# ZechengLi19/CIM

Measured on AMD Instinct MI355X. Metric: images/sec training step (ResNet-50 VOC, ~1k proposals/img) at 1/2/4/8 GPU, higher is better.
Workload: dtype fp32

## Files before the change

### cim_amd/csrc/conv1x1.hip

```cpp
#include "common.h"
#include "../../include/cim_hip.h"

#ifndef CIM_BODY_PRIO_LEVEL
#define CIM_BODY_PRIO_LEVEL 3
#endif
#if CIM_BODY_PRIO_LEVEL > 0
#define CIM_BODY_PRIO() __builtin_amdgcn_s_setprio(CIM_BODY_PRIO_LEVEL)
#else
#define CIM_BODY_PRIO()
#endif
namespace {

#ifndef CIM_SMALL_BK
#define CIM_SMALL_BK 32
#endif
#ifndef CIM_SMALL_ABL
#define CIM_SMALL_ABL 0
#endif
constexpr int SBM = 64, SBN = 64, SBK = CIM_SMALL_BK;
constexpr int SLD = 68;
typedef float f32x16 __attribute__((ext_vector_type(16)));
typedef float f32x4u __attribute__((ext_vector_type(4), aligned(4)));
__device__ __forceinline__ float4 ld4(const float* p) {
    const f32x4u v = *reinterpret_cast<const f32x4u*>(p);
    return make_float4(v.x, v.y, v.z, v.w);
}

struct SmallArgs {
    const float* A; const float* B; float* C; float* Xraw;
    const float* gamma; const float* beta; const float* mean; const float* var; const float* res;
    float eps;
    int M, N, K, lda, ldb, ldc;
    int a_mcontig, b_kcontig, relu, bn;
    int splits; float* ws;
    const float* colbias;
    const float* mask; const float* mgamma; const float* mvar; float meps;
    const float* mxr; const float* mmean; float* mpart; int mparts;
    int res_w, res_ws, res_hw;
};
struct InputBn { const float* y; const float* gamma; const float* var; float eps;
                 const float* xr; const float* mean; float* part; };

typedef unsigned int u32x4 __attribute__((ext_vector_type(4)));
typedef __amdgpu_buffer_rsrc_t rsrc_t;
__device__ __forceinline__ rsrc_t make_rsrc(const float* p, long long floats) {
    return __builtin_amdgcn_make_buffer_rsrc(const_cast<float*>(p), 0, (int)(unsigned)(floats * 4), 0x00020000);
}
__device__ __forceinline__ float4 bld4(rsrc_t r, unsigned byte_off) {
    const u32x4 v = __builtin_amdgcn_raw_buffer_load_b128(r, byte_off, 0, 0);
    return make_float4(__uint_as_float(v.x), __uint_as_float(v.y), __uint_as_float(v.z), __uint_as_float(v.w));
}
__device__ __forceinline__ float bld1(rsrc_t r, unsigned byte_off) {
    return __uint_as_float(__builtin_amdgcn_raw_buffer_load_b32(r, byte_off, 0, 0));
}
constexpr unsigned OOB = 0x7fffffffu;
__host__ __device__ __forceinline__ long long tile_extent(bool RC, int rows, int K, int ld) {
    return RC ? (long long)(K - 1) * ld + rows : (long long)(rows - 1) * ld + K;
}
template <bool RC, int ROWS>
__device__ __forceinline__ unsigned tile_off(int ld, int r0, int k0, int p) {
    int r, k;
    if (RC) { k = k0 + p / (ROWS / 4); r = r0 + (p % (ROWS / 4)) * 4; return ((unsigned)k * ld + r) * 4u; }
    r = r0 + p % ROWS; k = k0 + (p / ROWS) * 4;
    return ((unsigned)r * ld + k) * 4u;
}
template <bool RC, int ROWS>
__device__ __forceinline__ float4 tile_ktail(float4 v, int K, int k0, int p) {
    if (!RC) {
        const int left = K - (k0 + (p / ROWS) * 4);
        v.x = left > 0 ? v.x : 0.0f; v.y = left > 1 ? v.y : 0.0f; v.z = left > 2 ? v.z : 0.0f; v.w = left > 3 ? v.w : 0.0f;
    }
    return v;
}

template <bool RC, int ROWS>
__device__ __forceinline__ void tile_store(float* __restrict__ S, float4 v, int p) {
    if (RC) {
        const int k = p / (ROWS / 4), r = (p % (ROWS / 4)) * 4;
        *reinterpret_cast<float4*>(S + k * SLD + r) = v;
    } else {
        const int r = p % ROWS, k = (p / ROWS) * 4;
        S[(k + 0) * SLD + r] = v.x;
        S[(k + 1) * SLD + r] = v.y;
        S[(k + 2) * SLD + r] = v.z;
        S[(k + 3) * SLD + r] = v.w;
    }
}

__device__ __forceinline__ float small_value(const SmallArgs& g, int row, int col, float v, float& s1, float& s2) {
    const size_t o = (size_t)row * g.ldc + col;
    float y = v;
    if (g.bn) {
        const float a = g.gamma[row] * rsqrtf(g.var[row] + g.eps);
        y = fmaf(v, a, g.beta[row] - g.mean[row] * a);
    }
    if (g.res) {
        if (g.res_w == 0) y += g.res[o];
        else {
            const int py = col / g.res_w, px = col - py * g.res_w;
            if (!((py | px) & 1)) y += g.res[(size_t)row * g.res_hw + (py >> 1) * g.res_ws + (px >> 1)];
        }
    }
    if (g.colbias) y += g.colbias[col];
    if (g.relu) y = fmaxf(y, 0.0f);
    if (g.mask) {
        const bool on = g.mask[o] > 0.0f;
        if (g.mpart && on) { s1 += y; s2 = fmaf(y, g.mxr[o] - g.mmean[row], s2); }
        y = on ? y * (g.mgamma[row] * rsqrtf(g.mvar[row] + g.meps)) : 0.0f;
// ... 59 lines not shown
#pragma unroll
            for (int r = 0; r < 16; ++r) {
                const int row = row0 + 8 * (r >> 2) + 4 * (lane >> 5) + (r & 3);
                if (row < g.M) small_finish(g, row, col, acc[r]);
            }
        }
        return;
    }
#pragma unroll
    for (int r = 0; r < 16; ++r) {
        const int row = row0 + 8 * (r >> 2) + 4 * (lane >> 5) + (r & 3);
        float s1 = 0.0f, s2 = 0.0f;
        if (cm.in(nc) && row < g.M) small_finish(g, row, col, acc[r], s1, s2);
        small_put_part(g, row, cm.group(col0), lane, s1, s2);
    }
}


template <bool AM, bool BKc, int WN>
__global__ __launch_bounds__(128 * WN) void gemm_small_kernel(const SmallArgs g) {
    CIM_BODY_PRIO();
    constexpr int NT = 128 * WN, BNT = 32 * WN;
    constexpr int PA = SBM * 8 / NT, PB = BNT * 8 / NT;
    __shared__ __attribute__((aligned(16))) float As[2][SBK * SLD];
    __shared__ __attribute__((aligned(16))) float Bs[2][SBK * SLD];
    const int tid = threadIdx.x, lane = tid & 63, wave = tid >> 6;
    const int wm = wave / WN, wn = wave % WN;
    const int tiles_n = (g.N + BNT - 1) / BNT;
    const int tile = blockIdx.x;
    const int m0 = (tile / tiles_n) * SBM, n0 = (tile % tiles_n) * BNT;
    const int split = blockIdx.y;
    const int kper = ((g.K + g.splits - 1) / g.splits + SBK - 1) / SBK * SBK;
    const int kbeg = split * kper, kend = min(g.K, kbeg + kper);
#if CIM_SMALL_ABL == 4
    if (g.M > 0) return;
#endif

    f32x16 acc;
#pragma unroll
    for (int i = 0; i < 16; ++i) acc[i] = 0.0f;

    const rsrc_t RA_ = make_rsrc(g.A, tile_extent(AM, g.M, g.K, g.lda)), RB_ = make_rsrc(g.B, tile_extent(!BKc, g.N, g.K, g.ldb));
    unsigned oa[PA], ob[PB];
#pragma unroll
    for (int i = 0; i < PA; ++i) oa[i] = tile_off<AM, SBM>(g.lda, m0, kbeg, tid + i * NT);
#pragma unroll
    for (int i = 0; i < PB; ++i) ob[i] = tile_off<!BKc, BNT>(g.ldb, n0, kbeg, tid + i * NT);
    const unsigned sa = (AM ? (unsigned)g.lda * SBK : (unsigned)SBK) * 4u, sb = (!BKc ? (unsigned)g.ldb * SBK : (unsigned)SBK) * 4u;
    float4 ra0[PA], rb0[PB], ra1[PA], rb1[PB];
#if CIM_SMALL_ABL == 3
#define SM_GLOAD(RA, RB, S)                                                                                        \
    {                                                                                                              \
        _Pragma("unroll") for (int i = 0; i < PA; ++i) asm volatile("" : "+v"(RA[i].x), "+v"(RA[i].y), "+v"(RA[i].z), "+v"(RA[i].w)); \
        _Pragma("unroll") for (int i = 0; i < PB; ++i) asm volatile("" : "+v"(RB[i].x), "+v"(RB[i].y), "+v"(RB[i].z), "+v"(RB[i].w)); \
    }
#else
#define SM_GLOAD(RA, RB, S)                                                                                        \
    {                                                                                                              \
        _Pragma("unroll") for (int i = 0; i < PA; ++i) RA[i] = bld4(RA_, oa[i] + (unsigned)(S) * sa);               \
        _Pragma("unroll") for (int i = 0; i < PB; ++i) RB[i] = bld4(RB_, ob[i] + (unsigned)(S) * sb);               \
    }
#endif
#define SM_PUT(RA, RB, BUF, S)                                                                                     \
    {                                                                                                              \
        _Pragma("unroll") for (int i = 0; i < PA; ++i)                                                             \
            tile_store<AM, SBM>(As[BUF], tile_ktail<AM, SBM>(RA[i], g.K, kbeg + (S) * SBK, tid + i * NT), tid + i * NT);     \
        _Pragma("unroll") for (int i = 0; i < PB; ++i)                                                             \
            tile_store<!BKc, BNT>(Bs[BUF], tile_ktail<!BKc, BNT>(RB[i], g.K, kbeg + (S) * SBK, tid + i * NT), tid + i * NT); \
    }
#define SM_MMA(BUF)                                                                                                \
    {                                                                                                              \
        const float* __restrict__ a = As[BUF] + (lane >> 5) * SLD + wm * 32 + (lane & 31);                         \
        const float* __restrict__ b = Bs[BUF] + (lane >> 5) * SLD + wn * 32 + (lane & 31);                         \
        float av[SBK / 2], bv[SBK / 2];                                                                            \
        _Pragma("unroll") for (int t = 0; t < SBK / 2; ++t) { av[t] = a[2 * t * SLD]; bv[t] = b[2 * t * SLD]; }    \
        _Pragma("unroll") for (int t = 0; t < (CIM_SMALL_ABL == 1 ? 1 : SBK / 2); ++t)                             \
            acc = __builtin_amdgcn_mfma_f32_32x32x2f32(av[t], bv[t], acc, 0, 0, 0);                                \
        asm volatile("" : "+a"(acc));       \
    }
    if (kbeg < kend) {
        const int nslab = (kend - kbeg + SBK - 1) / SBK;
        const int last = nslab - 1;
        SM_GLOAD(ra0, rb0, 0)
        SM_GLOAD(ra1, rb1, min(1, last))
        SM_PUT(ra0, rb0, 0, 0)
        asm volatile("" : "+a"(acc));
        __syncthreads();
        for (int s = 0; s < nslab; s += 2) {
            SM_GLOAD(ra0, rb0, min(s + 2, last))
            SM_MMA(0)
            if (s + 1 < nslab) SM_PUT(ra1, rb1, 1, s + 1)
            __syncthreads();
            if (s + 1 >= nslab) break;
            SM_GLOAD(ra1, rb1, min(s + 3, last))
            SM_MMA(1)
            if (s + 2 < nslab) SM_PUT(ra0, rb0, 0, s + 2)
            __syncthreads();
        }
// ... 88 lines not shown
#pragma unroll
            for (int j = 0; j < 4; ++j) { t1 += a[j]; t2 += b[j]; }
        }
    }
    sh[0][grp][threadIdx.x & 31] = t1;
    sh[1][grp][threadIdx.x & 31] = t2;
    __syncthreads();
    if (grp == 0 && c < C) {
        float a1 = 0.0f, a2 = 0.0f;
#pragma unroll
        for (int k = 0; k < 8; ++k) { a1 += sh[0][k][threadIdx.x]; a2 += sh[1][k][threadIdx.x]; }
        if (d.dbeta) d.dbeta[c] = a1;
        if (d.dgamma) d.dgamma[c] = a2 * rsqrtf(d.var[c] + d.eps);
    }
}

enum { CONV_FWD = 0, CONV_DX = 1, CONV_DW = 2 };
struct ConvGeom { int H, W, Ho, Wo, stride, cin, cout; float inv_w; int dil; };

#ifndef CIM_CONV3_BK
#define CIM_CONV3_BK 32
#endif
constexpr int CBK = CIM_CONV3_BK;
template <int MODE, int KS = 3>
__global__ __launch_bounds__(256) void conv3x3_small_kernel(const SmallArgs g, const ConvGeom c) {
    CIM_BODY_PRIO();
    constexpr int TAPS = KS * KS;
    constexpr int NT = 256, PA = SBM * (CBK / 4) / NT, PB = SBN * (CBK / 4) / NT;
    extern __shared__ __attribute__((aligned(16))) float c3_smem[];
    float (*As)[CBK * SLD] = reinterpret_cast<float (*)[CBK * SLD]>(c3_smem);
    float (*Bs)[CBK * SLD] = reinterpret_cast<float (*)[CBK * SLD]>(c3_smem + 2 * CBK * SLD);
    const int tid = threadIdx.x, lane = tid & 63, wave = tid >> 6;
    const int wm = wave >> 1, wn = wave & 1;
    const int tiles_n = (g.N + SBN - 1) / SBN;
    const int m0 = (blockIdx.x / tiles_n) * SBM, n0 = (blockIdx.x % tiles_n) * SBN;
    const int split = blockIdx.y;
    const int kper = ((g.K + g.splits - 1) / g.splits + CBK - 1) / CBK * CBK;
    const int kbeg = split * kper, kend = min(g.K, kbeg + kper);

    const rsrc_t RA_ = make_rsrc(g.A, tile_extent(MODE == CONV_DX, g.M, g.K, g.lda));
    const rsrc_t RB_ = make_rsrc(g.B, (long long)(MODE == CONV_DX ? c.cout * c.Ho * c.Wo : c.cin * c.H * c.W));
    const int hw_src = MODE == CONV_DX ? c.Ho * c.Wo : c.H * c.W;
    int py[PB][4], px[PB][4];
    int boff[PB], bdy[PB], bdx[PB];
#pragma unroll
    for (int i = 0; i < PB; ++i) {
        const int p = tid + i * NT;
        if (MODE == CONV_DW) {
            const int n = n0 + p % SBN;
            const int ch = n / TAPS, tap = n - ch * TAPS;
            boff[i] = n < g.N ? ch * hw_src : -1;
            bdy[i] = (tap / KS - KS / 2) * c.dil;
            bdx[i] = (tap - (tap / KS) * KS - KS / 2) * c.dil;
        } else {
            const int wrow = (MODE == CONV_DX) ? c.W : c.Wo;
#pragma unroll
            for (int j = 0; j < 4; ++j) {
                const int n = n0 + (p % 16) * 4 + j;
                const int y = (int)(((float)n + 0.5f) * c.inv_w);
                py[i][j] = n < g.N ? y : -(1 << 20);
                px[i][j] = n - y * wrow;
            }
        }
    }
    unsigned oa[PA];
#pragma unroll
    for (int i = 0; i < PA; ++i) oa[i] = tile_off<MODE == CONV_DX, SBM>(g.lda, m0, kbeg, tid + i * NT);
    const unsigned sa = (MODE == CONV_DX ? (unsigned)g.lda * CBK : (unsigned)CBK) * 4u;

    auto load_b = [&](int k0, float4 (&rb)[PB]) {
#pragma unroll
        for (int i = 0; i < PB; ++i) {
            const int p = tid + i * NT;
            unsigned off[4];
            if (MODE == CONV_DW) {
                const int k = k0 + (p / SBN) * 4;
#pragma unroll
                for (int j = 0; j < 4; ++j) {
                    const int po = k + j;
                    const int yo = (int)(((float)po + 0.5f) * c.inv_w), xo = po - yo * c.Wo;
                    const int yi = yo * c.stride + bdy[i], xi = xo * c.stride + bdx[i];
                    const bool ok = boff[i] >= 0 && po < g.K && (unsigned)yi < (unsigned)c.H && (unsigned)xi < (unsigned)c.W;
                    off[j] = ok ? (unsigned)(boff[i] + yi * c.W + xi) * 4u : OOB;
                }
            } else {
                const int k = k0 + p / 16;
                const int ch = k / TAPS, tap = k - ch * TAPS;
                const int dy = (tap / KS - KS / 2) * c.dil, dx = (tap - (tap / KS) * KS - KS / 2) * c.dil;
                const int base = ch * hw_src;
#pragma unroll
                for (int j = 0; j < 4; ++j) {
                    if (MODE == CONV_DX) {
                        const int ty = py[i][j] - dy, tx = px[i][j] - dx;
                        const int yo = c.stride == 2 ? ty >> 1 : ty, xo = c.stride == 2 ? tx >> 1 : tx;
                        const bool ok = ty >= 0 && tx >= 0 && yo < c.Ho && xo < c.Wo && !(c.stride == 2 && ((ty | tx) & 1));
                        off[j] = ok ? (unsigned)(base + yo * c.Wo + xo) * 4u : OOB;
                    } else {
                        const int yi = py[i][j] * c.stride + dy, xi = px[i][j] * c.stride + dx;
                        const bool ok = (unsigned)yi < (unsigned)c.H && (unsigned)xi < (unsigned)c.W;
                        off[j] = ok ? (unsigned)(base + yi * c.W + xi) * 4u : OOB;
                    }
                }
            }
#if CIM_SMALL_ABL == 3
            asm volatile("" : "+v"(rb[i].x), "+v"(rb[i].y), "+v"(rb[i].z), "+v"(rb[i].w) : "v"(off[0]), "v"(off[1]), "v"(off[2]), "v"(off[3]));
#elif CIM_SMALL_ABL == 5
            rb[i] = make_float4(bld1(RB_, (unsigned)(p * 16 + k0 * 64)), bld1(RB_, (unsigned)(p * 16 + k0 * 64 + 4)),
                                bld1(RB_, (unsigned)(p * 16 + k0 * 64 + 8)), bld1(RB_, (unsigned)(p * 16 + k0 * 64 + 12)));
#else
            rb[i] = make_float4(bld1(RB_, off[0]), bld1(RB_, off[1]), bld1(RB_, off[2]), bld1(RB_, off[3]));
#endif
        }
    };
    auto load_a = [&](int s, float4 (&ra)[PA]) {
#pragma unroll
        for (int i = 0; i < PA; ++i)
            ra[i] = bld4(RA_, oa[i] + (unsigned)s * sa);
    };

    f32x16 acc;
#pragma unroll
    for (int i = 0; i < 16; ++i) acc[i] = 0.0f;
    float4 ra0[PA], rb0[PB], ra1[PA], rb1[PB];
#define C3_PUT(RA, RB, BUF, S)                                                                                      \
    {                                                                                                               \
        _Pragma("unroll") for (int i = 0; i < PA; ++i)                                                              \
            tile_store<MODE == CONV_DX, SBM>(As[BUF], tile_ktail<MODE == CONV_DX, SBM>(RA[i], g.K, kbeg + (S) * CBK, tid + i * NT), tid + i * NT); \
        _Pragma("unroll") for (int i = 0; i < PB; ++i) tile_store<MODE != CONV_DW, SBN>(Bs[BUF], RB[i], tid + i * NT); \
    }
#define C3_MMA(BUF)                                                                                                 \
    {                                                                                                               \
        const float* __restrict__ a = As[BUF] + (lane >> 5) * SLD + wm * 32 + (lane & 31);                          \
        const float* __restrict__ b = Bs[BUF] + (lane >> 5) * SLD + wn * 32 + (lane & 31);                          \
        float av[CBK / 2], bv[CBK / 2];                                                                             \
        _Pragma("unroll") for (int t = 0; t < CBK / 2; ++t) { av[t] = a[2 * t * SLD]; bv[t] = b[2 * t * SLD]; }     \
        _Pragma("unroll") for (int t = 0; t < (CIM_SMALL_ABL == 1 ? 1 : CBK / 2); ++t)                              \
            acc = __builtin_amdgcn_mfma_f32_32x32x2f32(av[t], bv[t], acc, 0, 0, 0);                                 \
        asm volatile("" : "+a"(acc));                                                                               \
    }
    if (kbeg < kend) {
        const int nslab = (kend - kbeg + CBK - 1) / CBK;
        const int last = nslab - 1;
        load_a(0, ra0); load_b(kbeg, rb0);
        load_a(min(1, last), ra1); load_b(kbeg + min(1, last) * CBK, rb1);
        C3_PUT(ra0, rb0, 0, 0)
        asm volatile("" : "+a"(acc));
        __syncthreads();
        for (int s = 0; s < nslab; s += 2) {
            load_a(min(s + 2, last), ra0); load_b(kbeg + min(s + 2, last) * CBK, rb0);
            C3_MMA(0)
            if (s + 1 < nslab) C3_PUT(ra1, rb1, 1, s + 1)
            __syncthreads();
            if (s + 1 >= nslab) break;
            load_a(min(s + 3, last), ra1); load_b(kbeg + min(s + 3, last) * CBK, rb1);
            C3_MMA(1)
            if (s + 2 < nslab) C3_PUT(ra0, rb0, 0, s + 2)
            __syncthreads();
        }
    }
#undef C3_PUT
#undef C3_MMA
    small_epilogue(g, acc, m0 + wm * 32, n0 + wn * 32, lane, split, ColIdentity{g.N});
}

struct Dx2Geom { int H, W, Ho, Wo, cin, cout; int first[5]; int tiles_n[4]; int group0[4]; };

__global__ __launch_bounds__(256) void conv3x3_dx2_kernel(const SmallArgs g, const Dx2Geom c) {
    CIM_BODY_PRIO();
    constexpr int NT = 256, PA = SBM * (CBK / 4) / NT, PB = SBN * (CBK / 4) / NT;
    extern __shared__ __attribute__((aligned(16))) float d2_smem[];
    float (*As)[CBK * SLD] = reinterpret_cast<float (*)[CBK * SLD]>(d2_smem);
    float (*Bs)[CBK * SLD] = reinterpret_cast<float (*)[CBK * SLD]>(d2_smem + 2 * CBK * SLD);
    const int tid = threadIdx.x, lane = tid & 63, wave = tid >> 6;
    const int wm = wave >> 1, wn = wave & 1;
    int cls = 0;
    while (cls < 3 && (int)blockIdx.x >= c.first[cls + 1]) ++cls;
    const int py = cls >> 1, px = cls & 1;
    const int Wc = (c.W - px + 1) >> 1, Nc = ((c.H - py + 1) >> 1) * Wc;
    const int local = (int)blockIdx.x - c.first[cls], tn = c.tiles_n[cls];
    const int m0 = (local / tn) * SBM, n0 = (local % tn) * SBN;
    const int nx = px ? 2 : 1, lgT = py + px, T = 1 << lgT;
    const int K = c.cout << lgT;
    const int nslab = (K + CBK - 1) / CBK;
    const int how = c.Ho * c.Wo;
    const rsrc_t RA_ = make_rsrc(g.A, tile_extent(true, g.M, 9 * c.cout, g.lda));
    const rsrc_t RB_ = make_rsrc(g.B, (long long)c.cout * how);
    int yc[PB][4], xc[PB][4];
#pragma unroll
    for (int i = 0; i < PB; ++i) {
        const int p = tid + i * NT;
#pragma unroll
        for (int j = 0; j < 4; ++j) {
            const int nc = n0 + (p % 16) * 4 + j;
            const int y = nc / Wc;
            yc[i][j] = nc < Nc ? y : -(1 << 20);
            xc[i][j] = nc - y * Wc;
        }
    }
    auto tap_of = [&](int j, int& tap, int& oy, int& ox) {
        const int jy = j / nx, jx = j - jy * nx;
        const int ky = py ? 2 * jy : 1, kx = px ? 2 * jx : 1;
        tap = ky * 3 + kx;
        oy = (py && jy == 0) ? 1 : 0;
        ox = (px && jx == 0) ? 1 : 0;
    };
    auto load_a = [&](int k0, float4 (&ra)[PA]) {
#pragma unroll
        for (int i = 0; i < PA; ++i) {
            const int p = tid + i * NT;
            const int k = k0 + p / (SBM / 4), r = m0 + (p % (SBM / 4)) * 4;
            const int co = k >> lgT;
            int tap, oy, ox;
            tap_of(k & (T - 1), tap, oy, ox);
            ra[i] = bld4(RA_, co < c.cout ? ((unsigned)(co * 9 + tap) * g.lda + r) * 4u : OOB);
        }
    };
    auto load_b = [&](int k0, float4 (&rb)[PB]) {
#pragma unroll
        for (int i = 0; i < PB; ++i) {
            const int p = tid + i * NT;
            const int k = k0 + p / 16;
            const int co = k >> lgT;
            int tap, oy, ox;
            tap_of(k & (T - 1), tap, oy, ox);
            const int base = co * how;
            unsigned off[4];
#pragma unroll
            for (int j = 0; j < 4; ++j) {
                const int yo = yc[i][j] + oy, xo = xc[i][j] + ox;
                const bool ok = co < c.cout && yo >= 0 && yo < c.Ho && xo < c.Wo;
                off[j] = ok ? (unsigned)(base + yo * c.Wo + xo) * 4u : OOB;
            }
            rb[i] = make_float4(bld1(RB_, off[0]), bld1(RB_, off[1]), bld1(RB_, off[2]), bld1(RB_, off[3]));
        }
    };
    f32x16 acc;
#pragma unroll
    for (int i = 0; i < 16; ++i) acc[i] = 0.0f;
    float4 ra0[PA], rb0[PB], ra1[PA], rb1[PB];
#define D2_PUT(RA, RB, BUF)                                                                                         \
    {                                                                                                               \
        _Pragma("unroll") for (int i = 0; i < PA; ++i) tile_store<true, SBM>(As[BUF], RA[i], tid + i * NT);          \
        _Pragma("unroll") for (int i = 0; i < PB; ++i) tile_store<true, SBN>(Bs[BUF], RB[i], tid + i * NT);          \
    }
#define D2_MMA(BUF)                                                                                                 \
    {                                                                                                               \
        const float* __restrict__ a = As[BUF] + (lane >> 5) * SLD + wm * 32 + (lane & 31);                          \
        const float* __restrict__ b = Bs[BUF] + (lane >> 5) * SLD + wn * 32 + (lane & 31);                          \
        float av[CBK / 2], bv[CBK / 2];                                                                             \
        _Pragma("unroll") for (int t = 0; t < CBK / 2; ++t) { av[t] = a[2 * t * SLD]; bv[t] = b[2 * t * SLD]; }     \
        _Pragma("unroll") for (int t = 0; t < CBK / 2; ++t)                                                         \
            acc = __builtin_amdgcn_mfma_f32_32x32x2f32(av[t], bv[t], acc, 0, 0, 0);                                 \
        asm volatile("" : "+a"(acc));                                                                               \
    }
    {
        const int last = nslab - 1;
        load_a(0, ra0); load_b(0, rb0);
        load_a(min(1, last) * CBK, ra1); load_b(min(1, last) * CBK, rb1);
        D2_PUT(ra0, rb0, 0)
        asm volatile("" : "+a"(acc));
        __syncthreads();
        for (int s = 0; s < nslab; s += 2) {
            load_a(min(s + 2, last) * CBK, ra0); load_b(min(s + 2, last) * CBK, rb0);
            D2_MMA(0)
            if (s + 1 < nslab) D2_PUT(ra1, rb1, 1)
            __syncthreads();
            if (s + 1 >= nslab) break;
            load_a(min(s + 3, last) * CBK, ra1); load_b(min(s + 3, last) * CBK, rb1);
            D2_MMA(1)
            if (s + 2 < nslab) D2_PUT(ra0, rb0, 0)
            __syncthreads();
        }
    }
// ... 54 lines not shown
    return 0;
}
static void launch_splitk_reduce(const SmallArgs& g, hipStream_t st) {
    if (g.mpart) {
        hipLaunchKernelGGL(small_splitk_reduce_rows_kernel, dim3((unsigned)((g.N + 255) / 256), (unsigned)g.M), dim3(256), 0, st, g);
    } else {
        const size_t n = (size_t)g.M * g.N;
        if (n >= (1u << 19) && g.ldc == g.N && n % 4 == 0 && (((size_t)g.ws | (size_t)g.C | (size_t)g.Xraw) & 15) == 0)
            hipLaunchKernelGGL(small_splitk_reduce4_kernel, dim3((unsigned)((n / 4 + 255) / 256)), dim3(256), 0, st, g);
        else
            hipLaunchKernelGGL(small_splitk_reduce_kernel, dim3((unsigned)((n + 255) / 256)), dim3(256), 0, st, g);
    }
}

template <bool AM, bool BKc>
static void launch_small(const SmallArgs& g, int splits, hipStream_t st, bool narrow) {
    const long long tm = (g.M + SBM - 1) / SBM;
    if (narrow)
        hipLaunchKernelGGL((gemm_small_kernel<AM, BKc, 1>), dim3((unsigned)(tm * ((g.N + 31) / 32)), (unsigned)splits), dim3(128), 0, st, g);
    else
        hipLaunchKernelGGL((gemm_small_kernel<AM, BKc, 2>), dim3((unsigned)(tm * ((g.N + 63) / 64)), (unsigned)splits), dim3(256), 0, st, g);
}

}

extern "C" int cim_gemm_small_splits(int M, int N, int K) {
    const long long tiles = (long long)((M + SBM - 1) / SBM) * ((N + SBN - 1) / SBN);
#ifndef CIM_SMALL_WGS
#define CIM_SMALL_WGS 512
#endif
#ifndef CIM_SMALL_MINSLABS
#define CIM_SMALL_MINSLABS 4
#endif
    constexpr int min_k = CIM_SMALL_MINSLABS * SBK, want = CIM_SMALL_WGS;
    int s = 1;
    while (tiles * s < want && K / (s * 2) >= min_k && s < 64) s *= 2;
    return s;
}

static int gemm_small_impl(const float* A, const float* B, float* C, int M, int N, int K, int lda, int ldb, int ldc,
                           int a_mcontig, int b_kcontig, float* x_raw, const float* gamma, const float* beta,
                           const float* mean, const float* var, float eps, const float* residual, int relu, int splits,
                           float* workspace, void* stream, const InputBn* in_bn, int res_w = 0) {
    CIM_CHECK_ARG(res_w == 0 || (residual && res_w > 0 && N % res_w == 0 && ldc == N));
    CIM_CHECK_ARG(A && B && C && M > 0 && N > 0 && K > 0 && lda > 0 && ldb > 0 && ldc >= N && splits >= 1);
    CIM_CHECK_ARG((gamma == nullptr) == (beta == nullptr) && (gamma == nullptr) == (mean == nullptr) && (gamma == nullptr) == (var == nullptr));
// ... 114 lines not shown
    if (rc) return rc;
    for (int b = 0; b < B && dx; ++b) {
        const InputBn ib{x + (size_t)b * cin * hw, in_gamma, in_var, in_eps, in_xr ? in_xr + (size_t)b * cin * hw : nullptr, in_mean,
                         in_part ? in_part + (size_t)b * 2 * ((hw + 31) / 32) * cin : nullptr};
        rc = gemm_small_impl(w, dconv + (size_t)b * cout * hw, dx + (size_t)b * cin * hw, cin, hw, cout, cin, hw, hw, 1, 0,
                             nullptr, nullptr, nullptr, nullptr, nullptr, 0.f, dx_add ? dx_add + (size_t)b * add_bs : nullptr, 0,
                             cim_gemm_small_splits(cin, hw, cout), ws_dx, stream, in_gamma ? &ib : nullptr, dx_add_w);
        if (rc) return rc;
    }
    if (join) fj.join();
    CIM_CHECK_LAUNCH();
    return 0;
}

namespace {
int conv3x3_launch(int mode, const float* A, const float* B, float* C, int M, int N, int K, int lda, int ldc, const ConvGeom& c,
                   float* x_raw, const float* gamma, const float* beta, const float* mean, const float* var, float eps,
                   const float* residual, int relu, int splits, float* ws, hipStream_t st, int ksize = 3, const InputBn* in_bn = nullptr) {
    SmallArgs g = small_args(A, B, C, M, N, K, lda, 0, ldc, splits, ws, in_bn, x_raw, gamma, beta, mean, var, eps, residual, relu);
    g.b_kcontig = mode == CONV_DW;
    const dim3 grid((unsigned)(((M + SBM - 1) / SBM) * ((N + SBN - 1) / SBN)), (unsigned)splits);
    auto kern = ksize == 7 ? conv3x3_small_kernel<CONV_FWD, 7>
                : mode == CONV_FWD ? conv3x3_small_kernel<CONV_FWD> : mode == CONV_DX ? conv3x3_small_kernel<CONV_DX> : conv3x3_small_kernel<CONV_DW>;
    const int rc = launch_lds(kern, grid, sizeof(float) * 4 * CBK * SLD, st, g, c);
    if (rc) return rc;
    if (splits > 1) launch_splitk_reduce(g, st);
    return 0;
}
ConvGeom conv_geom(int cin, int cout, int H, int W, int stride, int mode, int dil = 1) {
    ConvGeom c;
    c.H = H; c.W = W; c.stride = stride; c.cin = cin; c.cout = cout; c.dil = dil;
    c.Ho = (H - 1) / stride + 1; c.Wo = (W - 1) / stride + 1;
    c.inv_w = 1.0f / (float)(mode == CONV_DX ? W : c.Wo);
    return c;
}
}

#define CONV3_ARGS_OK(CIN_MULT)                                                                                      \
    CIM_CHECK_ARG(cin > 0 && cout > 0 && H > 0 && W > 0 && (stride == 1 || stride == 2) && W <= 4096 &&               \
                  dilation >= 1 && dilation <= 8 && (dilation == 1 || stride == 1) &&                                 \
                  (long long)H * W < (1ll << 20) && (long long)cin * H * W < (1ll << 29) && (long long)cout * H * W < (1ll << 29) && \
                  (long long)cin * cout * 9 < (1ll << 29) && cin % (CIN_MULT) == 0)

extern "C" int cim_conv3x3_nchw_splits(int cin, int cout, int H, int W, int stride) {
    const int Ho = (H - 1) / stride + 1, Wo = (W - 1) / stride + 1;
    return cim_gemm_small_splits(cout, Ho * Wo, 9 * cin);
}
// ... 125 lines not shown
    float* ws_dx = wt_own + (size_t)cout * cin * 9;
    float* ws_dw = ws_dx + (size_t)cim_gemm_small_splits(cin, hw, 9 * cout) * cin * hw;
    CIM_CHECK_ARG((size_t)cin * 9 * sizeof(float) <= 64 * 1024);
    int rc = dy_is_dconv ? 0 : cim_bn_act_bwd(dy, y, x_raw, gamma, mean, var, eps, dconv, dres, dgamma, dbeta, B, cout, hwo, relu, stream);
    if (rc) return rc;
    ForkJoin fj(st, cim::as_stream(side_stream), fork_event, join_event, dx && dw);
    hipStream_t st_dw = fj.fork();
    const int sp = cim_gemm_small_splits(cout, 9 * cin, hwo);
    rc = dw_over_images(B, dw, ws_dw, sp, (size_t)cout * cin * 9, st_dw, [&](int b, float* out) {
        return conv3x3_launch(CONV_DW, dconv + (size_t)b * cout * hwo, x + (size_t)b * cin * hw, out, cout, 9 * cin, hwo, hwo, 9 * cin, cw,
                              nullptr, nullptr, nullptr, nullptr, nullptr, 0.f, nullptr, 0, sp, ws_dw, st_dw);
    });
    if (rc) return rc;
    if (dx && !wt_ready) hipLaunchKernelGGL(conv3x3_wt_kernel, dim3(cout), dim3(256), sizeof(float) * cin * 9, st, w, wt_own, cin);
    const int parts = cim_conv3x3_dx_parts(H, W, dilation == 1 ? stride : 1);
    for (int b = 0; b < B && dx; ++b) {
        const InputBn ib{x + (size_t)b * cin * hw, in_gamma, in_var, in_eps, in_xr ? in_xr + (size_t)b * cin * hw : nullptr, in_mean,
                         in_part ? in_part + (size_t)b * 2 * parts * cin : nullptr};
        if (stride == 2 && dilation == 1) {
            SmallArgs g = small_args(wt, dconv + (size_t)b * cout * hwo, dx + (size_t)b * cin * hw, cin, hw, 9 * cout, cin, 0, hw, 1, nullptr,
                                     in_gamma ? &ib : nullptr);
            g.mparts = parts;
            const Dx2Geom c2 = dx2_geom(cin, cout, H, W);
            rc = launch_lds(conv3x3_dx2_kernel, dim3((unsigned)c2.first[4]), sizeof(float) * 4 * CBK * SLD, st, g, c2);
            if (rc) return rc;
            continue;
        }
        conv3x3_launch(CONV_DX, wt, dconv + (size_t)b * cout * hwo, dx + (size_t)b * cin * hw, cin, hw, 9 * cout, cin, hw, cx, nullptr,
                       nullptr, nullptr, nullptr, nullptr, 0.f, nullptr, 0, cim_gemm_small_splits(cin, hw, 9 * cout), ws_dx, st, 3,
                       in_gamma ? &ib : nullptr);
    }
    if (join) fj.join();
    CIM_CHECK_LAUNCH();
    return 0;
}
```

### include/cim_hip.h

```cpp
#ifndef CIM_HIP_H
#define CIM_HIP_H

#include <stdint.h>

#ifdef __cplusplus
extern "C" {
#endif

const char* cim_last_error(void);
int cim_abi_version(void);

int cim_roi_align_fwd(const float* feat, const float* rois, float* out,
                      int B, int C, int H, int W, int K, int P,
                      float spatial_scale, int sampling_ratio, int aligned, void* stream);

long long cim_roi_align_bwd_workspace(int K, int P, int H, int W);
int cim_roi_align_bwd(const float* grad_out, const float* rois, float* grad_in,
                      int B, int C, int H, int W, int K, int P,
                      float spatial_scale, int sampling_ratio, int aligned, float* workspace, void* stream);

int cim_roi_align_fwd_ws(const float* feat, const float* rois, float* out,
                         int B, int C, int H, int W, int K, int P,
                         float spatial_scale, int sampling_ratio, int aligned, float* workspace, void* stream);
int cim_roi_align_maskcat_fwd_ws(const float* feat, const float* rois, const float* masks, float* cat,
// ... 187 lines not shown
#define CIM_RESAMPLE_MAX_DST 4096
#define CIM_RESAMPLE_MAX_ASPECT 100
#define CIM_RESAMPLE_PRECISION_BITS 22
long long cim_resample_ws_bytes(int B, const int64_t* desc_host, int out_w, int out_h);
int cim_resample_tables(const int64_t* desc_host, const int64_t* desc_dev, int B, int out_w, int out_h, void* ws, void* stream);
int cim_resample_rgb(const uint8_t* src, const int64_t* desc_host, const int64_t* desc_dev, int B, int out_w, int out_h,
                     uint8_t* dst_u8, float* dst_f32, const float* mean_std6_host, void* ws, void* stream);

int cim_image_prep(const uint8_t* src_bgr, int h, int w, float* dst, int H, int W, long long plane_stride, int row_stride,
                   double inv_scale, int hflip, const float* mean_std6_host, void* stream);

int cim_maxpool2d_out_size(int in, int k, int stride, int pad);
int cim_maxpool2d_fwd(const float* x, float* y, int* idx, int NC, int H, int W, int k, int stride, int pad, void* stream);
int cim_maxpool2d_bwd(const float* dy, const int* idx, float* dx, int NC, int H, int W, int k, int stride, int pad, void* stream);
int cim_upsample_nearest_fwd(const float* x, float* y, int NC, int H, int W, int scale, int accumulate, void* stream);
int cim_upsample_nearest_bwd(const float* dy, float* dx, int NC, int H, int W, int scale, void* stream);

int cim_gemm_small_splits(int M, int N, int K);
int cim_gemm_small_f32(const float* A, const float* B, float* C, int M, int N, int K, int lda, int ldb, int ldc,
                       int a_mcontig, int b_kcontig, float* x_raw, const float* gamma, const float* beta,
                       const float* mean, const float* var, float eps, const float* residual, int relu, int splits,
                       float* workspace, void* stream);

long long cim_conv1x1_bwd_workspace(int B, int cin, int cout, int hw);
int cim_conv1x1_bn_act_bwd(const float* dy, const float* y, const float* x_raw, const float* x, const float* w,
                           const float* gamma, const float* mean, const float* var, float eps, int relu,
                           float* dres, float* dgamma, float* dbeta, float* dx, float* dw, int B, int cin, int cout, int hw,
                           float* workspace, void* stream, void* side_stream, void* fork_event, void* join_event, int join,
                           int dy_is_dconv, const float* in_gamma, const float* in_var, float in_eps,
                           const float* in_xr, const float* in_mean, float* in_part, const float* dx_add, int dx_add_w);
typedef struct { const float* part; const float* var; float eps; float* dgamma; float* dbeta; int images; int parts; int channels; } cim_bn_part_desc;
int cim_bn_part_finish(const cim_bn_part_desc* descs, int n, void* stream);

int cim_conv3x3_nchw_splits(int cin, int cout, int H, int W, int stride);
int cim_conv3x3_nchw_f32(const float* x, const float* w, float* y, int cin, int cout, int H, int W, int stride, int dilation,
                         float* x_raw, const float* gamma, const float* beta, const float* mean, const float* var, float eps,
                         const float* residual, int relu, int splits, float* workspace, void* stream);
int cim_conv7x7_nchw_f32(const float* x, const float* w, float* y, int cin, int cout, int H, int W, int stride,
                         const float* gamma, const float* beta, const float* mean, const float* var, float eps, int relu,
                         void* stream);
long long cim_conv3x3_nchw_bwd_workspace(int B, int cin, int cout, int H, int W, int stride);
int cim_conv3x3_dx_parts(int H, int W, int stride);
int cim_conv3x3_nchw_bn_act_bwd(const float* dy, const float* y, const float* x_raw, const float* x, const float* w,
                                const float* gamma, const float* mean, const float* var, float eps, int relu, float* dres,
                                float* dgamma, float* dbeta, float* dx, float* dw, int B, int cin, int cout, int H, int W,
                                int stride, int dilation, float* workspace, void* stream, void* side_stream, void* fork_event,
// ... 129 lines not shown
```

Baseline: 75.45.

## Swizzle LDS slab layout so MFMA fragments load as float4 chunks

Replaces the padded k-major LDS tile layout (stride 68) with a k-pair interleaved, XOR-swizzled slab, used by the small GEMM and the 3x3/dx2 conv kernels. Fragment reads for the 32x32x2 MFMA become four float4 LDS loads instead of sixteen scalar loads, and stores become float2 writes. The aim is fewer LDS instructions and fewer bank conflicts, plus a smaller LDS footprint. The cost is more complex index math for the global-to-LDS piece mapping, and test hooks are exported for the new mapping.

```diff
diff --git a/cim_amd/csrc/conv1x1.hip b/cim_amd/csrc/conv1x1.hip
--- a/cim_amd/csrc/conv1x1.hip
+++ b/cim_amd/csrc/conv1x1.hip
@@ -1,5 +1,6 @@
 #include "common.h"
 #include "../../include/cim_hip.h"
+#include "small_lds.h"
 
 #ifndef CIM_BODY_PRIO_LEVEL
 #define CIM_BODY_PRIO_LEVEL 3
@@ -18,7 +19,8 @@
 #define CIM_SMALL_ABL 0
 #endif
 constexpr int SBM = 64, SBN = 64, SBK = CIM_SMALL_BK;
-constexpr int SLD = 68;
+static_assert(SBK == small_lds::SLAB_K, "the LDS slab image (small_lds.h) is laid out for 32-k slabs");
+constexpr int STILE = SBM * SBK;
 typedef float f32x16 __attribute__((ext_vector_type(16)));
 typedef float f32x4u __attribute__((ext_vector_type(4), aligned(4)));
 __device__ __forceinline__ float4 ld4(const float* p) {
@@ -58,32 +60,55 @@
     return RC ? (long long)(K - 1) * ld + rows : (long long)(rows - 1) * ld + K;
 }
 template <bool RC, int ROWS>
-__device__ __forceinline__ unsigned tile_off(int ld, int r0, int k0, int p) {
+__device__ __forceinline__ void tile_piece(int tid, int i, int nt, int& r, int& k) {
+    if (RC) { small_lds::pair_rc(ROWS, tid + (i >> 1) * nt, r, k); k += 2 * (i & 1); }
+    else small_lds::piece_kc(ROWS, tid + i * nt, r, k);
+}
+template <bool RC, int ROWS>
+__device__ __forceinline__ unsigned tile_off(int ld, int r0, int k0, int tid, int i, int nt) {
     int r, k;
-    if (RC) { k = k0 + p / (ROWS / 4); r = r0 + (p % (ROWS / 4)) * 4; return ((unsigned)k * ld + r) * 4u; }
-    r = r0 + p % ROWS; k = k0 + (p / ROWS) * 4;
-    return ((unsigned)r * ld + k) * 4u;
-}
-template <bool RC, int ROWS>
-__device__ __forceinline__ float4 tile_ktail(float4 v, int K, int k0, int p) {
-    if (!RC) {
-        const int left = K - (k0 + (p / ROWS) * 4);
-        v.x = left > 0 ? v.x : 0.0f; v.y = left > 1 ? v.y : 0.0f; v.z = left > 2 ? v.z : 0.0f; v.w = left > 3 ? v.w : 0.0f;
-    }
+    tile_piece<RC, ROWS>(tid, i, nt, r, k);
+    r += r0; k += k0;
+    return RC ? ((unsigned)k * ld + r) * 4u : ((unsigned)r * ld + k) * 4u;
+}
+__device__ __forceinline__ float4 tile_ktail(float4 v, int left) {
+    v.x = left > 0 ? v.x : 0.0f; v.y = left > 1 ? v.y : 0.0f; v.z = left > 2 ? v.z : 0.0f; v.w = left > 3 ? v.w : 0.0f;
     return v;
 }
-
-template <bool RC, int ROWS>
-__device__ __forceinline__ void tile_store(float* __restrict__ S, float4 v, int p) {
+__device__ __forceinline__ void lds_put2(float* __restrict__ S, int slot, float lo, float hi) {
+    *reinterpret_cast<float2*>(S + slot) = make_float2(lo, hi);
+}
+__device__ __forceinline__ int tile_swap(int tid, int i, int nt) { return small_lds::pair_swap(tid + (i >> 1) * nt); }
+template <bool RC, int ROWS, int P, bool TAIL, bool SWAPPED = false>
+__device__ __forceinline__ void tile_put(float* __restrict__ S, const float4 (&v)[P], int K, int k0, int tid, int nt) {
+    static_assert(!RC || P % 2 == 0, "row-contiguous pieces are stored in pairs");
     if (RC) {
-        const int k = p / (ROWS / 4), r = (p % (ROWS / 4)) * 4;
-        *reinterpret_cast<float4*>(S + k * SLD + r) = v;
+#pragma unroll
+        for (int i = 0; i < P; i += 2) {
+            int r, k;
+            tile_piece<RC, ROWS>(tid, i, nt, r, k);
+            const int x = SWAPPED ? tile_swap(tid, i, nt) : 0;
+            const float a[4] = {v[i].x, v[i].y, v[i].z, v[i].w}, b[4] = {v[i + 1].x, v[i + 1].y, v[i + 1].z, v[i + 1].w};
+#pragma unroll
+            for (int j = 0; j < 4; ++j) lds_put2(S, small_lds::slot(ROWS, r + (j ^ x), k), a[j], b[j]);
+        }
     } else {
-        const int r = p % ROWS, k = (p / ROWS) * 4;
-        S[(k + 0) * SLD + r] = v.x;
-        S[(k + 1) * SLD + r] = v.y;
-        S[(k + 2) * SLD + r] = v.z;
-        S[(k + 3) * SLD + r] = v.w;
+#pragma unroll
+        for (int i = 0; i < P; ++i) {
+            int r, k;
+            tile_piece<RC, ROWS>(tid, i, nt, r, k);
+            const float4 w = TAIL ? tile_ktail(v[i], K - (k0 + k)) : v[i];
+            lds_put2(S, small_lds::slot(ROWS, r, k), w.x, w.z);
+            lds_put2(S, small_lds::slot(ROWS, r, k + 1), w.y, w.w);
+        }
+    }
+}
+template <int ROWS>
+__device__ __forceinline__ void tile_frag(const float* __restrict__ S, int r, int h, float (&f)[SBK / 2]) {
+#pragma unroll
+    for (int c = 0; c < SBK / 8; ++c) {
+        const float4 x = *reinterpret_cast<const float4*>(S + small_lds::frag_chunk(ROWS, r, h, c));
+        f[4 * c + 0] = x.x; f[4 * c + 1] = x.y; f[4 * c + 2] = x.z; f[4 * c + 3] = x.w;
     }
 }
 
@@ -189,8 +214,8 @@
     CIM_BODY_PRIO();
     constexpr int NT = 128 * WN, BNT = 32 * WN;
     constexpr int PA = SBM * 8 / NT, PB = BNT * 8 / NT;
-    __shared__ __attribute__((aligned(16))) float As[2][SBK * SLD];
-    __shared__ __attribute__((aligned(16))) float Bs[2][SBK * SLD];
+    __shared__ __attribute__((aligned(16))) float As[2][SBM * SBK];
+    __shared__ __attribute__((aligned(16))) float Bs[2][BNT * SBK];
     const int tid = threadIdx.x, lane = tid & 63, wave = tid >> 6;
     const int wm = wave / WN, wn = wave % WN;
     const int tiles_n = (g.N + BNT - 1) / BNT;
@@ -210,9 +235,9 @@
     const rsrc_t RA_ = make_rsrc(g.A, tile_extent(AM, g.M, g.K, g.lda)), RB_ = make_rsrc(g.B, tile_extent(!BKc, g.N, g.K, g.ldb));
     unsigned oa[PA], ob[PB];
 #pragma unroll
-    for (int i = 0; i < PA; ++i) oa[i] = tile_off<AM, SBM>(g.lda, m0, kbeg, tid + i * NT);
-#pragma unroll
-    for (int i = 0; i < PB; ++i) ob[i] = tile_off<!BKc, BNT>(g.ldb, n0, kbeg, tid + i * NT);
+    for (int i = 0; i < PA; ++i) oa[i] = tile_off<AM, SBM>(g.lda, m0, kbeg, tid, i, NT);
+#pragma unroll
+    for (int i = 0; i < PB; ++i) ob[i] = tile_off<!BKc, BNT>(g.ldb, n0, kbeg, tid, i, NT);
     const unsigned sa = (AM ? (unsigned)g.lda * SBK : (unsigned)SBK) * 4u, sb = (!BKc ? (unsigned)g.ldb * SBK : (unsigned)SBK) * 4u;
     float4 ra0[PA], rb0[PB], ra1[PA], rb1[PB];
 #if CIM_SMALL_ABL == 3
@@ -230,17 +255,14 @@
 #endif
 #define SM_PUT(RA, RB, BUF, S)                                                                                     \
     {                                                                                                              \
-        _Pragma("unroll") for (int i = 0; i < PA; ++i)                                                             \
-            tile_store<AM, SBM>(As[BUF], tile_ktail<AM, SBM>(RA[i], g.K, kbeg + (S) * SBK, tid + i * NT), tid + i * NT);     \
-        _Pragma("unroll") for (int i = 0; i < PB; ++i)                                                             \
-            tile_store<!BKc, BNT>(Bs[BUF], tile_ktail<!BKc, BNT>(RB[i], g.K, kbeg + (S) * SBK, tid + i * NT), tid + i * NT); \
+        tile_put<AM, SBM, PA, true>(As[BUF], RA, g.K, kbeg + (S) * SBK, tid, NT);                                   \
+        tile_put<!BKc, BNT, PB, true>(Bs[BUF], RB, g.K, kbeg + (S) * SBK, tid, NT);                                 \
     }
 #define SM_MMA(BUF)                                                                                                \
     {                                                                                                              \
-        const float* __restrict__ a = As[BUF] + (lane >> 5) * SLD + wm * 32 + (lane & 31);                         \
-        const float* __restrict__ b = Bs[BUF] + (lane >> 5) * SLD + wn * 32 + (lane & 31);                         \
         float av[SBK / 2], bv[SBK / 2];                                                                            \
-        _Pragma("unroll") for (int t = 0; t < SBK / 2; ++t) { av[t] = a[2 * t * SLD]; bv[t] = b[2 * t * SLD]; }    \
+        tile_frag<SBM>(As[BUF], wm * 32 + (lane & 31), lane >> 5, av);                                             \
+        tile_frag<BNT>(Bs[BUF], wn * 32 + (lane & 31), lane >> 5, bv);                                             \
         _Pragma("unroll") for (int t = 0; t < (CIM_SMALL_ABL == 1 ? 1 : SBK / 2); ++t)                             \
             acc = __builtin_amdgcn_mfma_f32_32x32x2f32(av[t], bv[t], acc, 0, 0, 0);                                \
         asm volatile("" : "+a"(acc));       \
@@ -375,14 +397,15 @@
 #define CIM_CONV3_BK 32
 #endif
 constexpr int CBK = CIM_CONV3_BK;
+static_assert(CBK == SBK, "one LDS slab image (small_lds.h) for the 1 x 1 and the 3 x 3 kernels");
 template <int MODE, int KS = 3>
 __global__ __launch_bounds__(256) void conv3x3_small_kernel(const SmallArgs g, const ConvGeom c) {
     CIM_BODY_PRIO();
     constexpr int TAPS = KS * KS;
     constexpr int NT = 256, PA = SBM * (CBK / 4) / NT, PB = SBN * (CBK / 4) / NT;
     extern __shared__ __attribute__((aligned(16))) float c3_smem[];
-    float (*As)[CBK * SLD] = reinterpret_cast<float (*)[CBK * SLD]>(c3_smem);
-    float (*Bs)[CBK * SLD] = reinterpret_cast<float (*)[CBK * SLD]>(c3_smem + 2 * CBK * SLD);
+    float (*As)[STILE] = reinterpret_cast<float (*)[STILE]>(c3_smem);
+    float (*Bs)[STILE] = reinterpret_cast<float (*)[STILE]>(c3_smem + 2 * STILE);
     const int tid = threadIdx.x, lane = tid & 63, wave = tid >> 6;
     const int wm = wave >> 1, wn = wave & 1;
     const int tiles_n = (g.N + SBN - 1) / SBN;
@@ -398,9 +421,10 @@
     int boff[PB], bdy[PB], bdx[PB];
 #pragma unroll
     for (int i = 0; i < PB; ++i) {
-        const int p = tid + i * NT;
+        int pr, pk;
+        tile_piece<MODE != CONV_DW, SBN>(tid, i, NT, pr, pk);
         if (MODE == CONV_DW) {
-            const int n = n0 + p % SBN;
+            const int n = n0 + pr;
             const int ch = n / TAPS, tap = n - ch * TAPS;
             boff[i] = n < g.N ? ch * hw_src : -1;
             bdy[i] = (tap / KS - KS / 2) * c.dil;
@@ -409,7 +433,7 @@
             const int wrow = (MODE == CONV_DX) ? c.W : c.Wo;
 #pragma unroll
             for (int j = 0; j < 4; ++j) {
-                const int n = n0 + (p % 16) * 4 + j;
+                const int n = n0 + pr + (j ^ tile_swap(tid, i, NT));
                 const int y = (int)(((float)n + 0.5f) * c.inv_w);
                 py[i][j] = n < g.N ? y : -(1 << 20);
                 px[i][j] = n - y * wrow;
@@ -418,16 +442,17 @@
     }
     unsigned oa[PA];
 #pragma unroll
-    for (int i = 0; i < PA; ++i) oa[i] = tile_off<MODE == CONV_DX, SBM>(g.lda, m0, kbeg, tid + i * NT);
+    for (int i = 0; i < PA; ++i) oa[i] = tile_off<MODE == CONV_DX, SBM>(g.lda, m0, kbeg, tid, i, NT);
     const unsigned sa = (MODE == CONV_DX ? (unsigned)g.lda * CBK : (unsigned)CBK) * 4u;
 
     auto load_b = [&](int k0, float4 (&rb)[PB]) {
 #pragma unroll
         for (int i = 0; i < PB; ++i) {
-            const int p = tid + i * NT;
+            int pr, pk;
+            tile_piece<MODE != CONV_DW, SBN>(tid, i, NT, pr, pk);
             unsigned off[4];
             if (MODE == CONV_DW) {
-                const int k = k0 + (p / SBN) * 4;
+                const int k = k0 + pk;
 #pragma unroll
                 for (int j = 0; j < 4; ++j) {
                     const int po = k + j;
@@ -437,7 +462,7 @@
                     off[j] = ok ? (unsigned)(boff[i] + yi * c.W + xi) * 4u : OOB;
                 }
             } else {
-                const int k = k0 + p / 16;
+                const int k = k0 + pk;
                 const int ch = k / TAPS, tap = k - ch * TAPS;
                 const int dy = (tap / KS - KS / 2) * c.dil, dx = (tap - (tap / KS) * KS - KS / 2) * c.dil;
                 const int base = ch * hw_src;
@@ -458,6 +483,7 @@
 #if CIM_SMALL_ABL == 3
             asm volatile("" : "+v"(rb[i].x), "+v"(rb[i].y), "+v"(rb[i].z), "+v"(rb[i].w) : "v"(off[0]), "v"(off[1]), "v"(off[2]), "v"(off[3]));
 #elif CIM_SMALL_ABL == 5
+            const int p = tid + i * NT;
             rb[i] = make_float4(bld1(RB_, (unsigned)(p * 16 + k0 * 64)), bld1(RB_, (unsigned)(p * 16 + k0 * 64 + 4)),
                                 bld1(RB_, (unsigned)(p * 16 + k0 * 64 + 8)), bld1(RB_, (unsigned)(p * 16 + k0 * 64 + 12)));
 #else
@@ -477,16 +503,14 @@
     float4 ra0[PA], rb0[PB], ra1[PA], rb1[PB];
 #define C3_PUT(RA, RB, BUF, S)                                                                                      \
     {                                                                                                               \
-        _Pragma("unroll") for (int i = 0; i < PA; ++i)                                                              \
-            tile_store<MODE == CONV_DX, SBM>(As[BUF], tile_ktail<MODE == CONV_DX, SBM>(RA[i], g.K, kbeg + (S) * CBK, tid + i * NT), tid + i * NT); \
-        _Pragma("unroll") for (int i = 0; i < PB; ++i) tile_store<MODE != CONV_DW, SBN>(Bs[BUF], RB[i], tid + i * NT); \
+        tile_put<MODE == CONV_DX, SBM, PA, true>(As[BUF], RA, g.K, kbeg + (S) * CBK, tid, NT);                       \
+        tile_put<MODE != CONV_DW, SBN, PB, false, true>(Bs[BUF], RB, g.K, 0, tid, NT);    \
     }
 #define C3_MMA(BUF)                                                                                                 \
     {                                                                                                               \
-        const float* __restrict__ a = As[BUF] + (lane >> 5) * SLD + wm * 32 + (lane & 31);                          \
-        const float* __restrict__ b = Bs[BUF] + (lane >> 5) * SLD + wn * 32 + (lane & 31);                          \
         float av[CBK / 2], bv[CBK / 2];                                                                             \
-        _Pragma("unroll") for (int t = 0; t < CBK / 2; ++t) { av[t] = a[2 * t * SLD]; bv[t] = b[2 * t * SLD]; }     \
+        tile_frag<SBM>(As[BUF], wm * 32 + (lane & 31), lane >> 5, av);                                              \
+        tile_frag<SBN>(Bs[BUF], wn * 32 + (lane & 31), lane >> 5, bv);                                              \
         _Pragma("unroll") for (int t = 0; t < (CIM_SMALL_ABL == 1 ? 1 : CBK / 2); ++t)                              \
             acc = __builtin_amdgcn_mfma_f32_32x32x2f32(av[t], bv[t], acc, 0, 0, 0);                                 \
         asm volatile("" : "+a"(acc));                                                                               \
@@ -522,8 +546,8 @@
     CIM_BODY_PRIO();
     constexpr int NT = 256, PA = SBM * (CBK / 4) / NT, PB = SBN * (CBK / 4) / NT;
     extern __shared__ __attribute__((aligned(16))) float d2_smem[];
-    float (*As)[CBK * SLD] = reinterpret_cast<float (*)[CBK * SLD]>(d2_smem);
-    float (*Bs)[CBK * SLD] = reinterpret_cast<float (*)[CBK * SLD]>(d2_smem + 2 * CBK * SLD);
+    float (*As)[STILE] = reinterpret_cast<float (*)[STILE]>(d2_smem);
+    float (*Bs)[STILE] = reinterpret_cast<float (*)[STILE]>(d2_smem + 2 * STILE);
     const int tid = threadIdx.x, lane = tid & 63, wave = tid >> 6;
     const int wm = wave >> 1, wn = wave & 1;
     int cls = 0;
@@ -541,10 +565,11 @@
     int yc[PB][4], xc[PB][4];
 #pragma unroll
     for (int i = 0; i < PB; ++i) {
-        const int p = tid + i * NT;
+        int pr, pk;
+        tile_piece<true, SBN>(tid, i, NT, pr, pk);
 #pragma unroll
         for (int j = 0; j < 4; ++j) {
-            const int nc = n0 + (p % 16) * 4 + j;
+            const int nc = n0 + pr + (j ^ tile_swap(tid, i, NT));
             const int y = nc / Wc;
             yc[i][j] = nc < Nc ? y : -(1 << 20);
             xc[i][j] = nc - y * Wc;
@@ -560,8 +585,9 @@
     auto load_a = [&](int k0, float4 (&ra)[PA]) {
 #pragma unroll
         for (int i = 0; i < PA; ++i) {
-            const int p = tid + i * NT;
-            const int k = k0 + p / (SBM / 4), r = m0 + (p % (SBM / 4)) * 4;
+            int pr, pk;
+            tile_piece<true, SBM>(tid, i, NT, pr, pk);
+            const int k = k0 + pk, r = m0 + pr;
             const int co = k >> lgT;
             int tap, oy, ox;
             tap_of(k & (T - 1), tap, oy, ox);
@@ -571,8 +597,9 @@
     auto load_b = [&](int k0, float4 (&rb)[PB]) {
 #pragma unroll
         for (int i = 0; i < PB; ++i) {
-            const int p = tid + i * NT;
-            const int k = k0 + p / 16;
+            int pr, pk;
+            tile_piece<true, SBN>(tid, i, NT, pr, pk);
+            const int k = k0 + pk;
             const int co = k >> lgT;
             int tap, oy, ox;
             tap_of(k & (T - 1), tap, oy, ox);
@@ -593,15 +620,14 @@
     float4 ra0[PA], rb0[PB], ra1[PA], rb1[PB];
 #define D2_PUT(RA, RB, BUF)                                                                                         \
     {                                                                                                               \
-        _Pragma("unroll") for (int i = 0; i < PA; ++i) tile_store<true, SBM>(As[BUF], RA[i], tid + i * NT);          \
-        _Pragma("unroll") for (int i = 0; i < PB; ++i) tile_store<true, SBN>(Bs[BUF], RB[i], tid + i * NT);          \
+        tile_put<true, SBM, PA, false>(As[BUF], RA, 0, 0, tid, NT);                                                  \
+        tile_put<true, SBN, PB, false, true>(Bs[BUF], RB, 0, 0, tid, NT);                                            \
     }
 #define D2_MMA(BUF)                                                                                                 \
     {                                                                                                               \
-        const float* __restrict__ a = As[BUF] + (lane >> 5) * SLD + wm * 32 + (lane & 31);                          \
-        const float* __restrict__ b = Bs[BUF] + (lane >> 5) * SLD + wn * 32 + (lane & 31);                          \
         float av[CBK / 2], bv[CBK / 2];                                                                             \
-        _Pragma("unroll") for (int t = 0; t < CBK / 2; ++t) { av[t] = a[2 * t * SLD]; bv[t] = b[2 * t * SLD]; }     \
+        tile_frag<SBM>(As[BUF], wm * 32 + (lane & 31), lane >> 5, av);                                              \
+        tile_frag<SBN>(Bs[BUF], wn * 32 + (lane & 31), lane >> 5, bv);                                              \
         _Pragma("unroll") for (int t = 0; t < CBK / 2; ++t)                                                         \
             acc = __builtin_amdgcn_mfma_f32_32x32x2f32(av[t], bv[t], acc, 0, 0, 0);                                 \
         asm volatile("" : "+a"(acc));                                                                               \
@@ -702,6 +728,19 @@
         hipLaunchKernelGGL((gemm_small_kernel<AM, BKc, 2>), dim3((unsigned)(tm * ((g.N + 63) / 64)), (unsigned)splits), dim3(256), 0, st, g);
 }
 
+}
+
+extern "C" int cim_small_lds_slot(int rows, int row, int k, int* slot) {
+    CIM_CHECK_ARG((rows == 32 || rows == 64) && row >= 0 && row < rows && k >= 0 && k < small_lds::SLAB_K && slot);
+    *slot = small_lds::slot(rows, row, k);
+    return 0;
+}
+extern "C" int cim_small_lds_piece(int rows, int row_contig, int index, int* row, int* k, int* row_xor) {
+    CIM_CHECK_ARG((rows == 32 || rows == 64) && row && k && row_xor && index >= 0 && index < (row_contig ? rows * 4 : rows * 8));
+    if (row_contig) small_lds::pair_rc(rows, index, *row, *k);
+    else small_lds::piece_kc(rows, index, *row, *k);
+    *row_xor = row_contig ? small_lds::pair_swap(index) : 0;
+    return 0;
 }
 
 extern "C" int cim_gemm_small_splits(int M, int N, int K) {
@@ -862,7 +901,7 @@
     const dim3 grid((unsigned)(((M + SBM - 1) / SBM) * ((N + SBN - 1) / SBN)), (unsigned)splits);
     auto kern = ksize == 7 ? conv3x3_small_kernel<CONV_FWD, 7>
                 : mode == CONV_FWD ? conv3x3_small_kernel<CONV_FWD> : mode == CONV_DX ? conv3x3_small_kernel<CONV_DX> : conv3x3_small_kernel<CONV_DW>;
-    const int rc = launch_lds(kern, grid, sizeof(float) * 4 * CBK * SLD, st, g, c);
+    const int rc = launch_lds(kern, grid, sizeof(float) * 4 * STILE, st, g, c);
     if (rc) return rc;
     if (splits > 1) launch_splitk_reduce(g, st);
     return 0;
@@ -1034,7 +1073,7 @@
                                      in_gamma ? &ib : nullptr);
             g.mparts = parts;
             const Dx2Geom c2 = dx2_geom(cin, cout, H, W);
-            rc = launch_lds(conv3x3_dx2_kernel, dim3((unsigned)c2.first[4]), sizeof(float) * 4 * CBK * SLD, st, g, c2);
+            rc = launch_lds(conv3x3_dx2_kernel, dim3((unsigned)c2.first[4]), sizeof(float) * 4 * STILE, st, g, c2);
             if (rc) return rc;
             continue;
         }
diff --git a/cim_amd/csrc/small_lds.h b/cim_amd/csrc/small_lds.h
--- /dev/null
+++ b/cim_amd/csrc/small_lds.h
@@ -0,0 +1,45 @@
+#pragma once
+
+#if defined(__HIPCC__) || defined(__CUDACC__)
+#define SMALL_LDS_FN __host__ __device__ __forceinline__
+#else
+#define SMALL_LDS_FN inline
+#endif
+
+namespace small_lds {
+
+constexpr int SLAB_K = 32;
+constexpr int RUN = SLAB_K / 2;
+
+SMALL_LDS_FN int slot(int rows, int r, int k) {
+    const int h = k & 1, t = k >> 1;
+    return h * rows * RUN + r * RUN + ((((t >> 2) ^ (r >> 2)) & 3) << 2) + (t & 3);
+}
+SMALL_LDS_FN int frag_chunk(int rows, int r, int h, int c) { return slot(rows, r, h + 8 * c); }
+
+SMALL_LDS_FN void piece_kc(int rows, int p, int& r, int& k0) {
+    r = (p & 1) | (((p >> 1) & 3) << 2) | (((p >> 4) & 1) << 1);
+    const int kb2 = (p >> 3) & 1;
+    int rest = p >> 5;
+    r |= (rest & 1) << 4;
+    rest >>= 1;
+    if (rows == 64) {
+        r |= (rest & 1) << 5;
+        rest >>= 1;
+    }
+    k0 = (kb2 << 2) | (rest << 3);
+}
+SMALL_LDS_FN void pair_rc(int rows, int q, int& r0, int& k) {
+    int quad = q & 7;
+    const int kb2 = (q >> 3) & 1;
+    int rest = q >> 4;
+    if (rows == 64) {
+        quad |= (rest & 1) << 3;
+        rest >>= 1;
+    }
+    r0 = quad * 4;
+    k = (rest & 1) | (kb2 << 2) | ((rest >> 1) << 3);
+}
+SMALL_LDS_FN int pair_swap(int q) { return (q >> 2) & 1; }
+
+}
diff --git a/include/cim_hip.h b/include/cim_hip.h
--- a/include/cim_hip.h
+++ b/include/cim_hip.h
@@ -233,6 +233,9 @@
                        const float* mean, const float* var, float eps, const float* residual, int relu, int splits,
                        float* workspace, void* stream);
 
+int cim_small_lds_slot(int rows, int row, int k, int* slot);
+int cim_small_lds_piece(int rows, int row_contig, int index, int* row, int* k, int* row_xor);
+
 long long cim_conv1x1_bwd_workspace(int B, int cin, int cout, int hw);
 int cim_conv1x1_bn_act_bwd(const float* dy, const float* y, const float* x_raw, const float* x, const float* w,
                            const float* gamma, const float* mean, const float* var, float eps, int relu,
```

Result: no change. 75.87 (median of 6 runs) (+0.6%).
